# shichaoy/pop_up_slam

Hardware: AMD Instinct MI355X
Metric: graph-solve iters/sec + final chi2, 1k-pose/5k-edge plane graph (higher is better)
Workload: dtype f64; 1 GPU; C2 synthetic corridor: 1000 SE3 poses, 200 planes, 5000 plane edges, 999 odometry edges (BASELINE.json configs[1], seed 42); jacobian_mode=numeric, total_lm_solves=773

## Files before the change

### pop_up_slam_amd/csrc/pps_api.cpp

```cpp
#include "pps_graph.h"

using namespace pps;
using namespace pps_impl;

namespace pps {
Switches read_switches() {
  auto on = [](const char* k) { return getenv(k) != nullptr; };
  auto num = [](const char* k, long long dflt) { const char* e = getenv(k); return e && *e ? atoll(e) : dflt; };
  Switches s;
  s.k1_thread_form = on("PPS_K1_THREAD_FORM");
  {
    long long plain = num("PPS_PLAIN_SCHEDULE", 0);
    if (on("PPS_PLAIN_SCHEDULE") && plain <= 0) plain = 15;
    s.no_preassemble = (plain & 1) != 0; s.no_solve_flow = (plain & 2) != 0; s.no_root_fuse = (plain & 4) != 0; s.split_expand = (plain & 8) != 0;
  }
  s.no_spec_lin = on("PPS_NO_SPEC_LIN");
  s.no_dual = on("PPS_NO_DUAL");
  s.no_strip = on("PPS_NO_STRIP");
  s.no_incremental = on("PPS_NO_INCREMENTAL");
  s.no_incr_compact = on("PPS_NO_INCR_COMPACT");
  s.verify_upload = on("PPS_DEBUG_VERIFY_UPLOAD");
  s.multi_levels = on("PPS_MULTI_LEVELS");
  s.multi_thread_form = on("PPS_MULTI_THREAD_FORM");
  s.debug_drop_flag = (int)num("PPS_DEBUG_DROP_FLAG", 0);
  if (on("PPS_DEBUG_DROP_FLAG") && s.debug_drop_flag < 1) s.debug_drop_flag = 1;
  s.trace = (int)num("PPS_TRACE", 0);
  if (on("PPS_TRACE") && s.trace < 1) s.trace = 1;
  {
    long long tm = num("PPS_TIMING", 0);
    if (on("PPS_TIMING") && tm <= 0) tm = 7;
    s.analysis_timing = (tm & 1) != 0; s.upload_timing = (tm & 2) != 0; s.multi_timing = (tm & 8) ? 2 : ((tm & 4) ? 1 : 0);
  }
  s.multi_split = (int)num("PPS_MULTI_SPLIT", 0);
  s.multi_thread_factors = num("PPS_MULTI_THREAD_FACTORS", 120000);
  return s;
}
}

namespace pps_impl {
void report_front_trace(pps_graph* g) {
  const Analysis& A = g->an;
  std::vector<long long> tr((size_t)A.n_fronts * 8);
  (void)hipMemcpy(tr.data(), g->dev.trace, tr.size() * 8, hipMemcpyDeviceToHost);
  if (g->dev.trace_solve) {
    for (int l = A.n_levels - 1; l >= 0; l--) {
      double ph[5] = {0, 0, 0, 0, 0}, gap = 0; int n = 0, ng = 0;
// ... 562 lines not shown
```

### pop_up_slam_amd/csrc/pps_device.h

```cpp
#pragma once

#include <hip/hip_runtime.h>

#include <cstdint>

#include "pps_cost.h"

namespace pps {

struct DevGraph {
  int n_pose = 0, n_plane = 0, pose_ld = 0, plane_ld = 0;
  double *pose_est = nullptr, *pose_lin = nullptr;
  double *plane_est = nullptr, *plane_lin = nullptr;
  int *pose_voff = nullptr, *plane_voff = nullptr;
  int n_obs = 0, n_odo = 0, n_pp = 0, n_lp = 0;
  int obs_ld = 0, odo_ld = 0, pp_ld = 0, lp_ld = 0;
  int *obs_pose = nullptr, *obs_plane = nullptr; double *obs_meas = nullptr, *obs_w = nullptr;
  int n_obs_fixed = 0; double* obs_ray = nullptr;
  int *odo_a = nullptr, *odo_b = nullptr;         double *odo_meas = nullptr, *odo_w = nullptr;
  int *pp_pose = nullptr;                          double *pp_meas = nullptr, *pp_w = nullptr;
  int *lp_plane = nullptr;                         double *lp_meas = nullptr, *lp_w = nullptr;
  double* J = nullptr;
  int64_t joff_obs = 0, joff_odo = 0, joff_pp = 0, joff_lp = 0;
  double* P = nullptr;
// ... 37 lines not shown
  double* chi2_partials = nullptr;
  int chi2_blocks = 0;
  double* dn_partials = nullptr;
  unsigned int* ticket = nullptr;
  double* result_dev = nullptr;
  long long* trace = nullptr;
  int trace_solve = 0;
  int no_strip = 0;
  unsigned sw = 0;
  double step_ac[4] = {0, 0, 0, 0};
  double* gwork = nullptr;
  int64_t gwork_stride = 0;
};

constexpr double kStatusInternal = 64.0;
enum : unsigned { SW_K1_THREAD_FORM = 1u, SW_NO_SOLVE_FLOW = 2u, SW_NO_ROOT_FUSE = 4u, SW_DEBUG_DROP_FLAG = 8u, SW_DEBUG_DROP_XFLAG = 16u };
struct Switches {
  bool k1_thread_form = false;
  bool no_preassemble = false;
  bool no_solve_flow = false;
  bool no_root_fuse = false;
  bool split_expand = false;
  bool no_spec_lin = false;
  bool no_dual = false;
  bool no_strip = false;
  bool no_incremental = false;
  bool no_incr_compact = false;
  bool verify_upload = false;
  bool multi_levels = false, multi_thread_form = false;
  int debug_drop_flag = 0;
  int trace = 0;
  bool analysis_timing = false, upload_timing = false;
  int multi_timing = 0;
  int multi_split = 0;
  long long multi_thread_factors = 120000;
  unsigned dev_bits() const {
    return (k1_thread_form ? SW_K1_THREAD_FORM : 0u) | (no_solve_flow ? SW_NO_SOLVE_FLOW : 0u) | (no_root_fuse ? SW_NO_ROOT_FUSE : 0u) |
           (debug_drop_flag == 1 ? SW_DEBUG_DROP_FLAG : 0u) | (debug_drop_flag == 2 ? SW_DEBUG_DROP_XFLAG : 0u);
  }
};
Switches read_switches();

struct LinGuard {
  const double* chi[2];
  const double* pose[2];
  const double* plane[2];
  double error;
  int on, single;
  int want = -1;
};

struct SpecLin {
  double *J, *P, *H, *Hf;
// ... 14 lines not shown
hipError_t launch_linearize(const DevGraph& d, int mode, bool at_estimate, hipStream_t st, const LinGuard* guard = nullptr, hipEvent_t ev0 = nullptr,
                            hipEvent_t ev1 = nullptr);
hipError_t launch_hblocks(const DevGraph& d, hipStream_t st, const LinGuard* guard = nullptr, bool products = true);
bool k1_lane_form(const DevGraph& d, int mode);
bool k1_products(const DevGraph& d, int mode);
hipError_t launch_factor_level(const DevGraph& d, int level_begin, int level_count, int level_max_front, double lambda,
                               hipStream_t st);
hipError_t launch_backsolve_level(const DevGraph& d, int level_begin, int level_count, hipStream_t st);
struct DualAlt {
  double *L, *U, *delta, *result_dev, *chi2_partials, *dn_partials;
  unsigned int* ticket;
  double lambda;
};
hipError_t launch_band_all(const DevGraph& d, const DualAlt* alt, int n_groups, int nwaves_factor, int nwaves_solve, int max_front, int max_panel,
                           int max_group_fronts, double lambda, int epoch, hipStream_t st, hipEvent_t ev0 = nullptr, hipEvent_t ev1 = nullptr);
int band_all_solve_waves(int max_panel, int max_group_fronts);
hipError_t launch_band_factor(const DevGraph& d, int grp_begin, int grp_count, int nwaves, int max_front, double lambda, hipStream_t st,
                              hipEvent_t ev0 = nullptr, hipEvent_t ev1 = nullptr, bool pre = false);
hipError_t launch_band_solve(const DevGraph& d, int grp_begin, int grp_count, int nwaves, int max_panel, int max_group_fronts, hipStream_t st,
                             const DualAlt* alt = nullptr);
hipError_t launch_band_factor_dual(const DevGraph& d, const DualAlt& alt, int grp_begin, int grp_count, int nwaves, int max_front, double lambda,
                                   hipStream_t st, hipEvent_t ev0 = nullptr, hipEvent_t ev1 = nullptr, bool pre = false);
bool band_root_fusable(const DevGraph& d, int grp_count, int max_front);
hipError_t launch_band_root(const DevGraph& d, const DualAlt* alt, int grp, int nwaves_factor, int nwaves_solve, int max_front, int max_panel,
                            int max_group_fronts, double lambda, hipStream_t st, hipEvent_t ev0 = nullptr, hipEvent_t ev1 = nullptr,
                            bool pre = false);
hipError_t launch_trial_dual(const DevGraph& d, const DualAlt& alt, const double* base_pose, const double* base_plane, double* out_pose0,
                             double* out_plane0, double* out_pose1, double* out_plane1, double* host_result0, double seq0, double* host_result1,
                             double seq1, hipStream_t st, int n_trials = 2);
hipError_t launch_trial_lin(const DevGraph& d, const DualAlt& alt, const SpecLin& sl, const double* base_pose, const double* base_plane, double* out_pose0,
// ... 94 lines not shown
```

### pop_up_slam_amd/csrc/pps_k3.hip

```cpp
#include <algorithm>
#include <atomic>
#include <cstdlib>

#include <hip/hip_ext.h>

#include "pps_kcommon.h"
#include "pps_regtile.h"
#include "pps_front_reg.h"

namespace pps {


constexpr int kLdsLimitBytes = 160 * 1024 - 1024;

int lds_front_limit() {
  int fa = 1;
  while ((size_t)(fa + 1) * ((fa + 1) | 1) * 8 <= (size_t)kLdsLimitBytes) fa++;
  return fa - 1;
}

template <bool USE_LDS>
__global__ __launch_bounds__(256) void k_front_factor(DevGraph d, int level_begin, double lambda) {
  extern __shared__ double lds[];
  const int s = d.level_fronts[level_begin + blockIdx.x];
// ... 1010 lines not shown
    if ((size_t)pws * want * sizeof(double) + flow_fixed <= (size_t)kLdsLimitBytes) nw = want; else flow = false;
  }
  const size_t bf = (size_t)pwf * nw * sizeof(double);
  const size_t bs = flow ? (size_t)pws * nw * sizeof(double) + flow_fixed : ((size_t)pws * nw + (size_t)max_group_fronts * kBandMaxRows) * sizeof(double);
  const size_t bytes = bf > bs ? bf : bs;
  const DualAlt a2 = alt ? *alt : DualAlt{};
  if (pre && flow) PPS_LAUNCH_EV(ev0, ev1, (k_band_root<true, true>), dim3(1, alt ? 2 : 1), dim3(64 * nw), bytes, st, d, a2, grp, lambda, pwf, pws, max_group_fronts);
  else if (pre) PPS_LAUNCH_EV(ev0, ev1, (k_band_root<true, false>), dim3(1, alt ? 2 : 1), dim3(64 * nw), bytes, st, d, a2, grp, lambda, pwf, pws, max_group_fronts);
  else if (flow) PPS_LAUNCH_EV(ev0, ev1, (k_band_root<false, true>), dim3(1, alt ? 2 : 1), dim3(64 * nw), bytes, st, d, a2, grp, lambda, pwf, pws, max_group_fronts);
  else PPS_LAUNCH_EV(ev0, ev1, (k_band_root<false, false>), dim3(1, alt ? 2 : 1), dim3(64 * nw), bytes, st, d, a2, grp, lambda, pwf, pws, max_group_fronts);
  return hipGetLastError();
}

hipError_t launch_band_all(const DevGraph& d, const DualAlt* alt, int n_groups, int nwaves_factor, int nwaves_solve, int max_front, int max_panel,
                           int max_group_fronts, double lambda, int epoch, hipStream_t st, hipEvent_t ev0, hipEvent_t ev1) {
  { const hipError_t e = ensure_band_attrs(); if (e != hipSuccess) return e; }
  const int pwf = (int)(band_lds_bytes(max_front, true) / sizeof(double)), pws = (int)(band_solve_lds_bytes(max_panel) / sizeof(double));
  const DualAlt a2 = alt ? *alt : DualAlt{};
  PPS_LAUNCH_EV(ev0, ev1, k_band_factor_all, dim3(n_groups, alt ? 2 : 1), dim3(64 * nwaves_factor), (size_t)pwf * nwaves_factor * sizeof(double), st, d, a2, lambda, pwf, epoch);
  const size_t fixed = ((size_t)max_group_fronts * kBandMaxRows + (size_t)(max_group_fronts + 1) / 2) * sizeof(double);
  PPS_LAUNCH(k_band_solve_all, dim3(n_groups, alt ? 2 : 1), dim3(64 * nwaves_solve), (size_t)pws * nwaves_solve * sizeof(double) + fixed, st, d, a2, n_groups, pws, max_group_fronts, epoch);
  return hipGetLastError();
}
int band_all_solve_waves(int max_panel, int max_group_fronts) {
  const size_t per_wave = band_solve_lds_bytes(max_panel);
  const size_t fixed = ((size_t)max_group_fronts * kBandMaxRows + (size_t)(max_group_fronts + 1) / 2) * sizeof(double);
  const size_t room = (size_t)kLdsLimitBytes > fixed ? ((size_t)kLdsLimitBytes - fixed) / per_wave : 0;
  return (int)std::min<size_t>(std::min<size_t>(12, (size_t)max_group_fronts), room);
}

__global__ __launch_bounds__(64) void k_front_solve(DevGraph d, int level_begin) {
  __shared__ double t[256];
  const int s = d.level_fronts[level_begin + blockIdx.x];
  const int p = d.f_p[s], b = d.f_b[s], f = p + b;
  const double* __restrict__ Lp = d.L + d.f_Loff[s];
  const int* __restrict__ bi = d.bidx + d.f_bidx_off[s];
// ... 340 lines not shown
```

### pop_up_slam_amd/csrc/pps_k4.hip

```cpp
#include <algorithm>
#include <cstdlib>

#include <hip/hip_ext.h>

#include "pps_geom.h"
#include "pps_kcommon.h"
#include "pps_k1_body.h"
#include "pps_k4_body.h"

namespace pps {

template <bool TRIAL>
__device__ __forceinline__ void body_retract(const DevGraph& d, double* __restrict__ pose_lin, double* __restrict__ pose_est,
                                             double* __restrict__ plane_lin, double* __restrict__ plane_est, int bx, double* red) {
  const int i = bx * blockDim.x + threadIdx.x;
  double dn = 0.0;
  if (i < d.n_pose) {
    double p[7], o[7], dl[6];
    load_pose(pose_lin, d.pose_ld, i, p);
    const int off = d.pose_voff[i];
#pragma unroll
    for (int k = 0; k < 6; k++) { dl[k] = d.delta[off + k]; dn += dl[k] * dl[k]; }
    pose_exmap(p, dl, o);
    if (TRIAL) {
// ... 40 lines not shown
}
hipError_t launch_retract_apply(const DevGraph& d, hipStream_t st) {
  const int n = d.n_pose + d.n_plane;
  if (n == 0) return hipSuccess;
  PPS_LAUNCH(k_retract<false>, dim3(cdiv(n, 256)), dim3(256), 0, st, d);
  return hipGetLastError();
}

__global__ __launch_bounds__(kChiBlock) void k_chi2(DevGraph d, const double* __restrict__ pose,
                                                    const double* __restrict__ plane, int nb_obs, int nb_odo, int nb_pp,
                                                    int n_dn, double* __restrict__ out, double seq) {
  body_chi2(d, pose, plane, nb_obs, nb_odo, nb_pp, n_dn, out, seq, blockIdx.x, gridDim.x);
}

__device__ __forceinline__ void body_retract_to(const DevGraph& d, const double* __restrict__ base_pose, const double* __restrict__ base_plane,
                                                double* __restrict__ out_pose, double* __restrict__ out_plane, int bx, double* red) {
  const int i = bx * blockDim.x + threadIdx.x;
  double dn = 0.0;
  if (i < d.n_pose) {
    double p[7], o[7], dl[6];
    load_pose(base_pose, d.pose_ld, i, p);
    const int off = d.pose_voff[i];
#pragma unroll
    for (int k = 0; k < 6; k++) { dl[k] = d.delta[off + k]; dn += dl[k] * dl[k]; }
    pose_exmap(p, dl, o);
#pragma unroll
    for (int k = 0; k < 7; k++) out_pose[(size_t)k * d.pose_ld + i] = o[k];
  } else if (i < d.n_pose + d.n_plane) {
    const int l = i - d.n_pose;
    double p[4], o[4], dl[3];
    load_plane(base_plane, d.plane_ld, l, p);
    const int off = d.plane_voff[l];
#pragma unroll
    for (int k = 0; k < 3; k++) { dl[k] = d.delta[off + k]; dn += dl[k] * dl[k]; }
    plane_exmap(p, dl, o);
#pragma unroll
    for (int k = 0; k < 4; k++) out_plane[(size_t)k * d.plane_ld + l] = o[k];
  }
#pragma unroll
  for (int o2 = 32; o2 > 0; o2 >>= 1) dn += __shfl_down(dn, o2, 64);
  if ((threadIdx.x & 63) == 0) red[threadIdx.x >> 6] = dn;
  __syncthreads();
  if (threadIdx.x == 0) d.dn_partials[bx] = red[0] + red[1] + red[2] + red[3];
}

__global__ __launch_bounds__(kChiBlock) void k_trial_dual(DevGraph d, DualAlt alt, const double* __restrict__ base_pose, const double* __restrict__ base_plane,
                                                          double* __restrict__ out_pose, double* __restrict__ out_plane, double* __restrict__ out_pose1,
                                                          double* __restrict__ out_plane1, int nb_ret, int nb_obs, int nb_odo, int nb_pp, int nb_chi,
                                                          double* __restrict__ out, double seq, double* __restrict__ out1, double seq1) {
  if (blockIdx.y) {
    d.delta = alt.delta; d.chi2_partials = alt.chi2_partials; d.dn_partials = alt.dn_partials; d.ticket = alt.ticket; d.result_dev = alt.result_dev;
    out_pose = out_pose1; out_plane = out_plane1; out = out1; seq = seq1;
  }
  const int total = nb_ret + nb_chi;
  if ((int)blockIdx.x >= nb_ret) {
    body_chi2<true, true>(d, base_pose, base_plane, nb_obs, nb_odo, nb_pp, nb_ret, out, seq, (int)blockIdx.x - nb_ret, nb_chi, total);
    return;
  }
// ... 32 lines not shown
                                                         double* __restrict__ out, double seq, double* __restrict__ out1, double seq1, int lb_obs, int lb_odo, int lb_pp, int apply) {
  static_assert(kChiBlock == kLanesPerBlock, "one block size for the trial blocks and the lane-form sweep");
  const int total = nb_ret + nb_chi;
  const bool sweep = (int)blockIdx.x >= 2 * total;
  const int y = sweep ? sl.which : ((int)blockIdx.x >= total ? 1 : 0);
  const int bx0 = sweep ? (int)blockIdx.x - 2 * total : (int)blockIdx.x - y * total;
  if (y) {
    d.delta = alt.delta; d.chi2_partials = alt.chi2_partials; d.dn_partials = alt.dn_partials; d.ticket = alt.ticket; d.result_dev = alt.result_dev;
    out_pose = out_pose1; out_plane = out_plane1; out = out1; seq = seq1;
  }
  if (sweep) {
    d.J = sl.J; d.P = sl.P; d.H = sl.H; d.Hf = sl.Hf;
    body_linearize_lanes(d, base_pose, base_plane, lb_obs, lb_odo, lb_pp, bx0, apply != 0);
    return;
  }
  if (bx0 >= nb_ret) {
    body_chi2<true, true>(d, base_pose, base_plane, nb_obs, nb_odo, nb_pp, nb_ret, out, seq, bx0 - nb_ret, nb_chi, total);
    return;
  }
  __shared__ double red[4];
  body_retract_to(d, base_pose, base_plane, out_pose, out_plane, bx0, red);
  __shared__ bool last;
  if (threadIdx.x == 0) {
    __builtin_amdgcn_fence(__ATOMIC_RELEASE, "agent");
    asm volatile("s_waitcnt vmcnt(0)" ::: "memory");
    last = atomicAdd(d.ticket, 1u) == (unsigned int)(total - 1);
  }
  __syncthreads();
  if (!last) return;
  if (threadIdx.x == 0) __builtin_amdgcn_fence(__ATOMIC_ACQUIRE, "agent");
  __syncthreads();
  chi2_finish(d, nb_chi, nb_ret, out, seq);
  if (threadIdx.x == 0) *d.ticket = 0u;
}

int trial_lin_waves(const DevGraph& d) {
  const int nb = cdiv(d.n_obs, kChiBlock) + cdiv(d.n_odo, kChiBlock) + cdiv(d.n_pp, kChiBlock) + cdiv(d.n_lp, kChiBlock) + cdiv(d.n_pose + d.n_plane, 256);
  const int lb = cdiv(d.n_obs_fixed, kObsPerBlock) + cdiv(d.n_odo, kFactorsPerBlock) + cdiv(d.n_pp, kFactorsPerBlock) + cdiv(d.n_lp, kFactorsPerBlock);
  return (2 * nb + lb) * (kChiBlock / 64);
}
bool trial_lin_ok(const DevGraph& d, int mode) { return k1_lane_form(d, mode) && d.n_obs == d.n_obs_fixed && d.P != nullptr; }

hipError_t launch_trial_lin(const DevGraph& d, const DualAlt& alt, const SpecLin& sl, const double* base_pose, const double* base_plane, double* out_pose0,
                            double* out_plane0, double* out_pose1, double* out_plane1, double* host_result0, double seq0, double* host_result1,
                            double seq1, hipStream_t st, hipEvent_t ev0, hipEvent_t ev1) {
  const int n = d.n_pose + d.n_plane;
  const int nb_obs = cdiv(d.n_obs, kChiBlock), nb_odo = cdiv(d.n_odo, kChiBlock), nb_pp = cdiv(d.n_pp, kChiBlock), nb_lp = cdiv(d.n_lp, kChiBlock);
// ... 180 lines not shown
```

### pop_up_slam_amd/csrc/pps_k4_body.h

```cpp
#pragma once
#include "pps_cost.h"
#include "pps_geom.h"
#include "pps_kcommon.h"

namespace pps {

constexpr int kChiBlock = 256;

__device__ __forceinline__ void chi2_finish(const DevGraph& d, int nb, int n_dn, double* __restrict__ out, double seq) {
  double cs = 0.0, dn = 0.0;
  for (int i = threadIdx.x; i < nb; i += kChiBlock) cs += __hip_atomic_load(&d.chi2_partials[i], __ATOMIC_RELAXED, __HIP_MEMORY_SCOPE_AGENT);
  for (int i = threadIdx.x; i < n_dn; i += kChiBlock) dn += __hip_atomic_load(&d.dn_partials[i], __ATOMIC_RELAXED, __HIP_MEMORY_SCOPE_AGENT);
#pragma unroll
  for (int o = 32; o > 0; o >>= 1) { cs += __shfl_down(cs, o, 64); dn += __shfl_down(dn, o, 64); }
  __shared__ double red2[2][kChiBlock / 64];
  if ((threadIdx.x & 63) == 0) { red2[0][threadIdx.x >> 6] = cs; red2[1][threadIdx.x >> 6] = dn; }
  __syncthreads();
  if (threadIdx.x == 0) {
    double a = 0.0, b2 = 0.0;
    for (int k = 0; k < kChiBlock / 64; k++) { a += red2[0][k]; b2 += red2[1][k]; }
    const double npd = __hip_atomic_load(&d.result_dev[2], __ATOMIC_RELAXED, __HIP_MEMORY_SCOPE_AGENT);
    d.result_dev[0] = a; d.result_dev[1] = b2; d.result_dev[2] = 0.0;
    out[0] = a; out[1] = b2; out[2] = npd;
    __hip_atomic_store(&out[3], seq, __ATOMIC_RELEASE, __HIP_MEMORY_SCOPE_SYSTEM);
  }
}

template <bool TICKET = true, bool APPLY = false, bool ROBUST = false>
__device__ __forceinline__ void body_chi2(const DevGraph& d, const double* __restrict__ pose,
                                          const double* __restrict__ plane, int nb_obs, int nb_odo, int nb_pp,
                                          int n_dn, double* __restrict__ out, double seq, int bx, int nb, int total_blocks = 0, const CostFn& cost = CostFn{}) {
  __shared__ double red[kChiBlock / 64];
  int b = bx;
  double s = 0.0;
  if (b < nb_obs) {
    const int i = b * kChiBlock + threadIdx.x;
    if (i < d.n_obs) {
      double pz[7], pl[4], ms[4], w[6], e[3], r[3];
      fetch_pose<APPLY>(d, pose, d.obs_pose[i], pz);
      fetch_plane<APPLY>(d, plane, d.obs_plane[i], pl);
      if (i < d.n_obs_fixed) load_soa<4>(d.obs_meas, d.obs_ld, i, ms);
      else {
        double ray[6];
        load_soa<6>(d.obs_ray, d.n_obs - d.n_obs_fixed, i - d.n_obs_fixed, ray);
        repop_wall_plane(pz, ray, ms);
      }
// ... 44 lines not shown
      s = r[0] * r[0] + r[1] * r[1] + r[2] * r[2];
    }
  }
#pragma unroll
  for (int o = 32; o > 0; o >>= 1) s += __shfl_down(s, o, 64);
  if ((threadIdx.x & 63) == 0) red[threadIdx.x >> 6] = s;
  __syncthreads();
  if (!TICKET) {
    if (threadIdx.x == 0) { double t = 0.0; for (int k = 0; k < kChiBlock / 64; k++) t += red[k]; d.chi2_partials[bx] = t; }
    return;
  }
  __shared__ bool last;
  if (threadIdx.x == 0) {
    double t = 0.0;
    for (int k = 0; k < kChiBlock / 64; k++) t += red[k];
    d.chi2_partials[bx] = t;
    __builtin_amdgcn_fence(__ATOMIC_RELEASE, "agent");
    asm volatile("s_waitcnt vmcnt(0)" ::: "memory");
    last = atomicAdd(d.ticket, 1u) == (unsigned int)((total_blocks > 0 ? total_blocks : nb) - 1);
  }
  __syncthreads();
  if (!last) return;
  if (threadIdx.x == 0) __builtin_amdgcn_fence(__ATOMIC_ACQUIRE, "agent");
  __syncthreads();
  chi2_finish(d, nb, n_dn, out, seq);
  if (threadIdx.x == 0) *d.ticket = 0u;
}

}
```

### pop_up_slam_amd/csrc/pps_lm.h

```cpp
#pragma once
#include <cmath>
#include <cstdio>
#include <vector>

#include "../../include/pps.h"

namespace pps_impl {

struct LmSink {
  const pps_props* prop;
  std::vector<double>*tr_lambda, *tr_chi2;
  std::vector<int>* tr_acc;
  pps_stats* stats;
  bool verbose;
};

enum class LmVerdict { Rejected, Accepted, Converged };

constexpr const char* kLmNotPdMessage = "normal equations not positive definite at the last LM trial";

struct LmControl {
  double lambda, error = 0.0, dnorm = 0.0;
  int num_iter = 0;
  bool last_notpd = false;
  int n_notpd = 0;

  explicit LmControl(const pps_props& p) : lambda(p.lm_lambda0) {}

  bool running(const pps_props& p) const { return (p.max_iterations <= 0 || num_iter < p.max_iterations) && dnorm > p.epsilon2 && error > p.epsilon_abs; }

  void take_step(const double* rec) {
    dnorm = std::sqrt(rec[1]);
    last_notpd = rec[2] != 0.0;
    n_notpd += last_notpd ? 1 : 0;
  }

  __attribute__((always_inline)) LmVerdict judge(const LmSink& s, double error_new) {
    const pps_props& p = *s.prop;
    num_iter++;
    const double error_diff = error - error_new;
    const bool accepted = error_diff > 0.;
    s.tr_lambda->push_back(lambda); s.tr_chi2->push_back(error_new); s.tr_acc->push_back(accepted ? 1 : 0);
    if (s.verbose) fprintf(stderr, "LM Iteration %d: (lambda=%g) %s %.12g\n", num_iter, lambda, accepted ? "residual:" : "rejected", error_new);
    if (!accepted) {
      s.stats->lm_trials_rejected++;
      lambda *= p.lm_lambda_factor;
      return LmVerdict::Rejected;
    }
    s.stats->lm_trials_accepted++;
    const bool converged = error_diff < p.epsilon_rel * error;
    error = error_new;
    if (converged) return LmVerdict::Converged;
    lambda /= p.lm_lambda_factor;
    return LmVerdict::Accepted;
  }

  int finish(const LmSink& s, int* iterations) const {
    pps_stats& st = *s.stats;
    st.lm_iterations = num_iter;
    st.chi2_final = error; st.lambda_final = lambda; st.last_delta_norm = dnorm;
    st.lm_trials_notpd = n_notpd;
    if (iterations) *iterations = num_iter;
    return last_notpd ? PPS_ENOTPD : PPS_OK;
  }
};

}
```

### pop_up_slam_amd/csrc/pps_solve.cpp

```cpp
#include "pps_graph.h"

using namespace pps;
using namespace pps_impl;

namespace pps_impl {

struct PhaseTimer {
  pps_graph* g; double* acc; bool on;
  PhaseTimer(pps_graph* g_, double* a) : g(g_), acc(a), on(g_->profiling >= 2) { if (on) (void)hipEventRecord(g->ev[0], g->stream); }
  ~PhaseTimer() {
    if (!on) return;
    (void)hipEventRecord(g->ev[1], g->stream);
    (void)hipEventSynchronize(g->ev[1]);
    float ms = 0;
    (void)hipEventElapsedTime(&ms, g->ev[0], g->ev[1]);
    *acc += 1e-3 * ms;
  }
};

int do_linearize(pps_graph* g, const LinGuard* guard = nullptr) {
  if (g->profiling == 1) {
    if (g->k1_used + 2 > (int)g->k1_events.size()) {
      for (int k = 0; k < 2; k++) { hipEvent_t e; HIP_TRY(g, hipEventCreate(&e)); g->k1_events.push_back(e); }
    }
    g->k1_skip.resize(g->k1_events.size() / 2, 0);
    g->k1_skip[g->k1_used / 2] = 0;
    HIP_TRY(g, lin_launch(g, g->props.jacobian_mode, false, guard, g->k1_events[g->k1_used], g->k1_events[g->k1_used + 1]));
    g->k1_used += 2;
  } else
  { PhaseTimer t(g, &g->stats.t_linearize); HIP_TRY(g, lin_launch(g, g->props.jacobian_mode, false, guard)); }
  { PhaseTimer t(g, &g->stats.t_assemble); HIP_TRY(g, launch_hblocks(g->dev, g->stream, guard, k1_products(g->dev, g->props.jacobian_mode))); }
  if (!guard) g->stats.n_linearize++;
  return PPS_OK;
}

static int enqueue_factor_solve(pps_graph* g, const DevGraph& dv, const DualAlt* alt, double lambda, hipStream_t st_, bool events) {
  const Analysis& A = g->an;
  if (g->k3_all) {
    hipEvent_t e0 = nullptr, e1 = nullptr;
    if (events) {
      if (g->fk_used + 2 > (int)g->fk_events.size()) for (int k = 0; k < 2; k++) { hipEvent_t e; HIP_TRY(g, hipEventCreate(&e)); g->fk_events.push_back(e); }
      e0 = g->fk_events[g->fk_used]; e1 = g->fk_events[g->fk_used + 1]; g->fk_used += 2;
    }
    g->k3_epoch = g->k3_epoch >= (1 << 30) ? 1 : g->k3_epoch + 1;
    HIP_TRY(g, launch_band_all(dv, alt, A.n_groups, g->k3_nw_factor, g->k3_nw_solve, g->k3_max_front, g->k3_max_panel, g->k3_max_grp, lambda, g->k3_epoch, st_, e0, e1));
    return PPS_OK;
  }
  const int top = A.n_stages - 1;
  const bool fuse = top >= 0 && band_root_fusable(dv, A.stage_grp_off[top + 1] - A.stage_grp_off[top], A.stage_max_front[top]);
  for (int st = 0; st < A.n_stages; st++) {
    hipEvent_t e0 = nullptr, e1 = nullptr;
    if (events) {
      if (g->fk_used + 2 > (int)g->fk_events.size()) for (int k = 0; k < 2; k++) { hipEvent_t e; HIP_TRY(g, hipEventCreate(&e)); g->fk_events.push_back(e); }
      e0 = g->fk_events[g->fk_used]; e1 = g->fk_events[g->fk_used + 1]; g->fk_used += 2;
    }
    const int g0 = A.stage_grp_off[st], ng = A.stage_grp_off[st + 1] - g0;
    const bool pre = st < (int)g->stage_pre.size() && g->stage_pre[st] != 0;
    if (fuse && st == top)
      HIP_TRY(g, launch_band_root(dv, alt, g0, g->stage_nw_factor[st], g->stage_nw_solve[st], A.stage_max_front[st], g->stage_max_panel[st],
                                  g->stage_max_grp_fronts[st], lambda, st_, e0, e1, pre));
    else if (alt) HIP_TRY(g, launch_band_factor_dual(dv, *alt, g0, ng, g->stage_nw_factor[st], A.stage_max_front[st], lambda, st_, e0, e1, pre));
    else HIP_TRY(g, launch_band_factor(dv, g0, ng, g->stage_nw_factor[st], A.stage_max_front[st], lambda, st_, e0, e1, pre));
  }
  for (int st = fuse ? top - 1 : top; st >= 0; st--)
    HIP_TRY(g, launch_band_solve(dv, A.stage_grp_off[st], A.stage_grp_off[st + 1] - A.stage_grp_off[st], g->stage_nw_solve[st],
                                 g->stage_max_panel[st], g->stage_max_grp_fronts[st], st_, alt));
  return PPS_OK;
}

int do_solve_on(pps_graph* g, const DevGraph& dv, double lambda, hipStream_t st_) { return enqueue_factor_solve(g, dv, nullptr, lambda, st_, false); }
// ... 269 lines not shown
    const SpecLin sl{g->spec_J, g->spec_P, g->spec_H, g->spec_Hf, pred_launched};
    hipEvent_t e0 = nullptr, e1 = nullptr;
    fused_pair = -1;
    if (g->profiling == 1) {
      if (g->k1_used + 2 > (int)g->k1_events.size()) for (int k = 0; k < 2; k++) { hipEvent_t e; HIP_TRY(g, hipEventCreate(&e)); g->k1_events.push_back(e); }
      g->k1_skip.resize(g->k1_events.size() / 2, 0);
      fused_pair = g->k1_used / 2;
      g->k1_skip[fused_pair] = 1;
      e0 = g->k1_events[g->k1_used]; e1 = g->k1_events[g->k1_used + 1]; g->k1_used += 2;
    }
    HIP_TRY(g, launch_trial_lin(d, alt, sl, d.pose_lin, d.plane_lin, t_pose[0], t_plane[0], t_pose[1], t_plane[1], slot[0], s0, slot[1], s1, g->stream, e0, e1));
    const LinGuard gd{{d.result_dev, g->spec_result}, {nullptr, nullptr}, {nullptr, nullptr}, lm.error, error_known ? 1 : 0, use_alt ? 0 : 1, pred_launched};
    HIP_TRY(g, launch_hblocks_spec(d, sl, g->stream, &gd));
    return PPS_OK;
  };
  auto enqueue_dual = [&](double lam) -> int {
    DualAlt alt{g->spec_L, g->spec_U, g->spec_delta, g->spec_result, g->spec_chi2_partials, g->spec_dn_partials, g->spec_ticket,
                lam * prop.lm_lambda_factor};
    have_next = use_alt;
    const int n_trials = use_alt ? 2 : 1;
    { const int rc2 = enqueue_factor_solve(g, d, use_alt ? &alt : nullptr, lam, g->stream, g->profiling == 1); if (rc2 != PPS_OK) return rc2; }
    g->stats.n_factorize += n_trials;
    g->seq += 1.0; seqs[0] = g->seq;
    g->seq2 += 1.0; seqs[1] = g->seq2;
    if (fuse_lin) return enqueue_trial_lin(alt, seqs[0], seqs[1]);
    HIP_TRY(g, launch_trial_dual(d, alt, d.pose_lin, d.plane_lin, t_pose[0], t_plane[0], t_pose[1], t_plane[1], slot[0], seqs[0], slot[1], seqs[1],
                                 g->stream, n_trials));
    return PPS_OK;
  };
  rc = do_linearize(g); if (rc != PPS_OK) return rc;
  g->seq += 1.0;
  const double seq0 = g->seq;
  HIP_TRY(g, launch_chi2(d, false, slot0, seq0, g->stream));
  const bool spec_lin = !g->sw.no_spec_lin && !fuse_lin && !adaptive;
  int spec_pair = -1;
  auto enqueue_spec_lin = [&](double err) -> int {
// ... 1 lines not shown
    LinGuard gd{{d.result_dev, g->spec_result}, {t_pose[0], t_pose[1]}, {t_plane[0], t_plane[1]}, err, 1, have_next ? 0 : 1};
    spec_pair = g->profiling == 1 ? g->k1_used / 2 : -1;
    return do_linearize(g, &gd);
  };
  auto drop_spec_lin = [&]() { if (spec_pair >= 0 && (size_t)spec_pair < g->k1_skip.size()) g->k1_skip[spec_pair] = 1; spec_pair = -1; };
  rc = enqueue_dual(lm.lambda); if (rc != PPS_OK) return rc;
  rc = wait_result(g, slot0, seq0); if (rc != PPS_OK) return rc;
  lm.error = slot0[0]; error_known = true;
  g->stats.chi2_initial = lm.error;
  rc = enqueue_spec_lin(lm.error); if (rc != PPS_OK) return rc;
  rc = wait_result(g, slot[0], seqs[0]); if (rc != PPS_OK) return rc;
  int cur = 0;
  lm.take_step(slot[0]);
  bool trial_taken = false;
  while (lm.running(prop)) {
    const LmVerdict v = lm.judge(sink, slot[cur][0]);
    if (v == LmVerdict::Converged) { trial_taken = true; break; }
    if (v == LmVerdict::Accepted) {
      if (adaptive) use_alt = cur != 0;
      pred = cur;
      std::swap(d.pose_lin, t_pose[cur]); std::swap(d.plane_lin, t_plane[cur]);
      if (fuse_lin && cur == pred_launched) {
        std::swap(d.J, g->spec_J); std::swap(d.P, g->spec_P); std::swap(d.H, g->spec_H); std::swap(d.Hf, g->spec_Hf);
        g->stats.n_linearize++;
        if (fused_pair >= 0 && (size_t)fused_pair < g->k1_skip.size()) g->k1_skip[fused_pair] = 0;
      }
      else if (fuse_lin) { rc = do_linearize(g); if (rc != PPS_OK) return rc; }
      else if (spec_lin) { g->stats.n_linearize++; spec_pair = -1; }
      else { rc = do_linearize(g); if (rc != PPS_OK) return rc; }
      rc = enqueue_dual(lm.lambda); if (rc != PPS_OK) return rc;
      rc = enqueue_spec_lin(lm.error); if (rc != PPS_OK) return rc;
      cur = 0;
      rc = wait_result(g, slot[0], seqs[0]); if (rc != PPS_OK) return rc;
    } else {
      if (have_next) {
        cur = 1; have_next = false;
        rc = wait_result(g, slot[1], seqs[1]); if (rc != PPS_OK) return rc;
      } else {
        drop_spec_lin();
        if (adaptive) use_alt = true;
        rc = enqueue_dual(lm.lambda); if (rc != PPS_OK) return rc;
        rc = enqueue_spec_lin(lm.error); if (rc != PPS_OK) return rc;
        cur = 0;
        rc = wait_result(g, slot[0], seqs[0]); if (rc != PPS_OK) return rc;
      }
    }
    lm.take_step(slot[cur]);
  }
  drop_spec_lin();
  if (trial_taken) { std::swap(d.pose_lin, t_pose[cur]); std::swap(d.plane_lin, t_plane[cur]); }
  d.pose_est = d.pose_lin; d.plane_est = d.plane_lin;
  d.pose_lin = t_pose[0]; d.plane_lin = t_plane[0];
  g->spec_pose = t_pose[1]; g->spec_plane = t_plane[1];
  return end_lm_solve(g, lm, sink, iterations, t0);
}

static int lm_solve(pps_graph* g, int* iterations) {
  const double t0 = now_s();
  begin_solve(g);
  int rc = prepare_solve(g);
  if (rc != PPS_OK) return rc;
  if (g->use_band && g->profiling < 2 && !g->dev.trace && !g->sw.no_dual && !robust(g)) return lm_solve_dual(g, iterations, t0);
  const pps_props& prop = g->props;
  if (!g->status_clean) HIP_TRY(g, launch_clear_status(g->dev, g->stream));
// ... 99 lines not shown
```

Baseline: 17090 LM iters/s.

## Defer LM bookkeeping past factor launch and lighten chi2 result publishing

Splits the LM judge into a decision step and a deferred record step, so the trace and stats bookkeeping runs after the band-factor kernel is launched rather than before it. The band_all launch is split into a precomputed plan plus separate factor and solve launches, so the host starts the GPU work sooner on the critical path. On the device side, the trial and chi2 kernels publish partial sums through relaxed atomic exchanges instead of stores plus release fences, raise wave priority, and write the host-visible result with relaxed stores ordered by a waitcnt. This trades formal memory-ordering guarantees for lower fence latency. An optional timing mode reports the host gap between recording a trial and launching the factor kernel.

Result: faster. 17410 LM iters/s (median of 6 runs) (+1.9%).

```diff
diff --git a/pop_up_slam_amd/csrc/pps_api.cpp b/pop_up_slam_amd/csrc/pps_api.cpp
--- a/pop_up_slam_amd/csrc/pps_api.cpp
+++ b/pop_up_slam_amd/csrc/pps_api.cpp
@@ -16,6 +16,8 @@
   }
   s.no_spec_lin = on("PPS_NO_SPEC_LIN");
   s.no_dual = on("PPS_NO_DUAL");
+  s.lm_plain_host = on("PPS_LM_PLAIN_HOST");
+  s.no_early_record = on("PPS_NO_EARLY_RECORD");
   s.no_strip = on("PPS_NO_STRIP");
   s.no_incremental = on("PPS_NO_INCREMENTAL");
   s.no_incr_compact = on("PPS_NO_INCR_COMPACT");
@@ -30,6 +32,7 @@
     long long tm = num("PPS_TIMING", 0);
     if (on("PPS_TIMING") && tm <= 0) tm = 7;
     s.analysis_timing = (tm & 1) != 0; s.upload_timing = (tm & 2) != 0; s.multi_timing = (tm & 8) ? 2 : ((tm & 4) ? 1 : 0);
+    s.lm_timing = (tm & 16) != 0;
   }
   s.multi_split = (int)num("PPS_MULTI_SPLIT", 0);
   s.multi_thread_factors = num("PPS_MULTI_THREAD_FACTORS", 120000);
diff --git a/pop_up_slam_amd/csrc/pps_device.h b/pop_up_slam_amd/csrc/pps_device.h
--- a/pop_up_slam_amd/csrc/pps_device.h
+++ b/pop_up_slam_amd/csrc/pps_device.h
@@ -75,7 +75,7 @@
 };
 
 constexpr double kStatusInternal = 64.0;
-enum : unsigned { SW_K1_THREAD_FORM = 1u, SW_NO_SOLVE_FLOW = 2u, SW_NO_ROOT_FUSE = 4u, SW_DEBUG_DROP_FLAG = 8u, SW_DEBUG_DROP_XFLAG = 16u };
+enum : unsigned { SW_K1_THREAD_FORM = 1u, SW_NO_SOLVE_FLOW = 2u, SW_NO_ROOT_FUSE = 4u, SW_DEBUG_DROP_FLAG = 8u, SW_DEBUG_DROP_XFLAG = 16u, SW_NO_EARLY_RECORD = 32u };
 struct Switches {
   bool k1_thread_form = false;
   bool no_preassemble = false;
@@ -84,6 +84,8 @@
   bool split_expand = false;
   bool no_spec_lin = false;
   bool no_dual = false;
+  bool no_early_record = false;
+  bool lm_plain_host = false;
   bool no_strip = false;
   bool no_incremental = false;
   bool no_incr_compact = false;
@@ -91,13 +93,14 @@
   bool multi_levels = false, multi_thread_form = false;
   int debug_drop_flag = 0;
   int trace = 0;
-  bool analysis_timing = false, upload_timing = false;
+  bool analysis_timing = false, upload_timing = false, lm_timing = false;
   int multi_timing = 0;
   int multi_split = 0;
   long long multi_thread_factors = 120000;
   unsigned dev_bits() const {
     return (k1_thread_form ? SW_K1_THREAD_FORM : 0u) | (no_solve_flow ? SW_NO_SOLVE_FLOW : 0u) | (no_root_fuse ? SW_NO_ROOT_FUSE : 0u) |
-           (debug_drop_flag == 1 ? SW_DEBUG_DROP_FLAG : 0u) | (debug_drop_flag == 2 ? SW_DEBUG_DROP_XFLAG : 0u);
+           (debug_drop_flag == 1 ? SW_DEBUG_DROP_FLAG : 0u) | (debug_drop_flag == 2 ? SW_DEBUG_DROP_XFLAG : 0u) |
+           (no_early_record ? SW_NO_EARLY_RECORD : 0u);
   }
 };
 Switches read_switches();
@@ -142,6 +145,11 @@
 };
 hipError_t launch_band_all(const DevGraph& d, const DualAlt* alt, int n_groups, int nwaves_factor, int nwaves_solve, int max_front, int max_panel,
                            int max_group_fronts, double lambda, int epoch, hipStream_t st, hipEvent_t ev0 = nullptr, hipEvent_t ev1 = nullptr);
+struct BandAllPlan { int n_groups, nw_factor, nw_solve, pwf, pws, max_group_fronts; size_t lds_factor, lds_solve; };
+hipError_t band_all_plan(int n_groups, int nwaves_factor, int nwaves_solve, int max_front, int max_panel, int max_group_fronts, BandAllPlan* p);
+hipError_t launch_band_all_factor(const DevGraph& d, const DualAlt* alt, const BandAllPlan& p, double lambda, int epoch, hipStream_t st,
+                                  hipEvent_t ev0 = nullptr, hipEvent_t ev1 = nullptr);
+hipError_t launch_band_all_solve(const DevGraph& d, const DualAlt* alt, const BandAllPlan& p, int epoch, hipStream_t st);
 int band_all_solve_waves(int max_panel, int max_group_fronts);
 hipError_t launch_band_factor(const DevGraph& d, int grp_begin, int grp_count, int nwaves, int max_front, double lambda, hipStream_t st,
                               hipEvent_t ev0 = nullptr, hipEvent_t ev1 = nullptr, bool pre = false);
diff --git a/pop_up_slam_amd/csrc/pps_k3.hip b/pop_up_slam_amd/csrc/pps_k3.hip
--- a/pop_up_slam_amd/csrc/pps_k3.hip
+++ b/pop_up_slam_amd/csrc/pps_k3.hip
@@ -1048,12 +1048,29 @@
 
 hipError_t launch_band_all(const DevGraph& d, const DualAlt* alt, int n_groups, int nwaves_factor, int nwaves_solve, int max_front, int max_panel,
                            int max_group_fronts, double lambda, int epoch, hipStream_t st, hipEvent_t ev0, hipEvent_t ev1) {
+  BandAllPlan p;
+  { const hipError_t e = band_all_plan(n_groups, nwaves_factor, nwaves_solve, max_front, max_panel, max_group_fronts, &p); if (e != hipSuccess) return e; }
+  { const hipError_t e = launch_band_all_factor(d, alt, p, lambda, epoch, st, ev0, ev1); if (e != hipSuccess) return e; }
+  return launch_band_all_solve(d, alt, p, epoch, st);
+}
+hipError_t band_all_plan(int n_groups, int nwaves_factor, int nwaves_solve, int max_front, int max_panel, int max_group_fronts, BandAllPlan* p) {
   { const hipError_t e = ensure_band_attrs(); if (e != hipSuccess) return e; }
-  const int pwf = (int)(band_lds_bytes(max_front, true) / sizeof(double)), pws = (int)(band_solve_lds_bytes(max_panel) / sizeof(double));
+  p->n_groups = n_groups; p->nw_factor = nwaves_factor; p->nw_solve = nwaves_solve; p->max_group_fronts = max_group_fronts;
+  p->pwf = (int)(band_lds_bytes(max_front, true) / sizeof(double)); p->pws = (int)(band_solve_lds_bytes(max_panel) / sizeof(double));
+  p->lds_factor = (size_t)p->pwf * nwaves_factor * sizeof(double);
+  const size_t fixed = ((size_t)max_group_fronts * kBandMaxRows + (size_t)(max_group_fronts + 1) / 2) * sizeof(double);
+  p->lds_solve = (size_t)p->pws * nwaves_solve * sizeof(double) + fixed;
+  return hipSuccess;
+}
+hipError_t launch_band_all_factor(const DevGraph& d, const DualAlt* alt, const BandAllPlan& p, double lambda, int epoch, hipStream_t st, hipEvent_t ev0,
+                                  hipEvent_t ev1) {
   const DualAlt a2 = alt ? *alt : DualAlt{};
-  PPS_LAUNCH_EV(ev0, ev1, k_band_factor_all, dim3(n_groups, alt ? 2 : 1), dim3(64 * nwaves_factor), (size_t)pwf * nwaves_factor * sizeof(double), st, d, a2, lambda, pwf, epoch);
-  const size_t fixed = ((size_t)max_group_fronts * kBandMaxRows + (size_t)(max_group_fronts + 1) / 2) * sizeof(double);
-  PPS_LAUNCH(k_band_solve_all, dim3(n_groups, alt ? 2 : 1), dim3(64 * nwaves_solve), (size_t)pws * nwaves_solve * sizeof(double) + fixed, st, d, a2, n_groups, pws, max_group_fronts, epoch);
+  PPS_LAUNCH_EV(ev0, ev1, k_band_factor_all, dim3(p.n_groups, alt ? 2 : 1), dim3(64 * p.nw_factor), p.lds_factor, st, d, a2, lambda, p.pwf, epoch);
+  return hipGetLastError();
+}
+hipError_t launch_band_all_solve(const DevGraph& d, const DualAlt* alt, const BandAllPlan& p, int epoch, hipStream_t st) {
+  const DualAlt a2 = alt ? *alt : DualAlt{};
+  PPS_LAUNCH(k_band_solve_all, dim3(p.n_groups, alt ? 2 : 1), dim3(64 * p.nw_solve), p.lds_solve, st, d, a2, p.n_groups, p.pws, p.max_group_fronts, epoch);
   return hipGetLastError();
 }
 int band_all_solve_waves(int max_panel, int max_group_fronts) {
diff --git a/pop_up_slam_amd/csrc/pps_k4.hip b/pop_up_slam_amd/csrc/pps_k4.hip
--- a/pop_up_slam_amd/csrc/pps_k4.hip
+++ b/pop_up_slam_amd/csrc/pps_k4.hip
@@ -78,7 +78,7 @@
 }
 
 __device__ __forceinline__ void body_retract_to(const DevGraph& d, const double* __restrict__ base_pose, const double* __restrict__ base_plane,
-                                                double* __restrict__ out_pose, double* __restrict__ out_plane, int bx, double* red) {
+                                                double* __restrict__ out_pose, double* __restrict__ out_plane, int bx, double* red, bool light = false) {
   const int i = bx * blockDim.x + threadIdx.x;
   double dn = 0.0;
   if (i < d.n_pose) {
@@ -105,7 +105,10 @@
   for (int o2 = 32; o2 > 0; o2 >>= 1) dn += __shfl_down(dn, o2, 64);
   if ((threadIdx.x & 63) == 0) red[threadIdx.x >> 6] = dn;
   __syncthreads();
-  if (threadIdx.x == 0) d.dn_partials[bx] = red[0] + red[1] + red[2] + red[3];
+  if (threadIdx.x == 0) {
+    const double t = red[0] + red[1] + red[2] + red[3];
+    if (light) publish_partial(&d.dn_partials[bx], t); else d.dn_partials[bx] = t;
+  }
 }
 
 __global__ __launch_bounds__(kChiBlock) void k_trial_dual(DevGraph d, DualAlt alt, const double* __restrict__ base_pose, const double* __restrict__ base_plane,
@@ -168,15 +171,17 @@
     body_linearize_lanes(d, base_pose, base_plane, lb_obs, lb_odo, lb_pp, bx0, apply != 0);
     return;
   }
+  const bool light = (d.sw & SW_NO_EARLY_RECORD) == 0;
+  if (light) __builtin_amdgcn_s_setprio(3);
   if (bx0 >= nb_ret) {
-    body_chi2<true, true>(d, base_pose, base_plane, nb_obs, nb_odo, nb_pp, nb_ret, out, seq, bx0 - nb_ret, nb_chi, total);
+    body_chi2<true, true>(d, base_pose, base_plane, nb_obs, nb_odo, nb_pp, nb_ret, out, seq, bx0 - nb_ret, nb_chi, total, CostFn{}, light);
     return;
   }
   __shared__ double red[4];
-  body_retract_to(d, base_pose, base_plane, out_pose, out_plane, bx0, red);
+  body_retract_to(d, base_pose, base_plane, out_pose, out_plane, bx0, red, light);
   __shared__ bool last;
   if (threadIdx.x == 0) {
-    __builtin_amdgcn_fence(__ATOMIC_RELEASE, "agent");
+    if (!light) __builtin_amdgcn_fence(__ATOMIC_RELEASE, "agent");
     asm volatile("s_waitcnt vmcnt(0)" ::: "memory");
     last = atomicAdd(d.ticket, 1u) == (unsigned int)(total - 1);
   }
@@ -184,7 +189,7 @@
   if (!last) return;
   if (threadIdx.x == 0) __builtin_amdgcn_fence(__ATOMIC_ACQUIRE, "agent");
   __syncthreads();
-  chi2_finish(d, nb_chi, nb_ret, out, seq);
+  chi2_finish(d, nb_chi, nb_ret, out, seq, light);
   if (threadIdx.x == 0) *d.ticket = 0u;
 }
 
diff --git a/pop_up_slam_amd/csrc/pps_k4_body.h b/pop_up_slam_amd/csrc/pps_k4_body.h
--- a/pop_up_slam_amd/csrc/pps_k4_body.h
+++ b/pop_up_slam_amd/csrc/pps_k4_body.h
@@ -7,7 +7,14 @@
 
 constexpr int kChiBlock = 256;
 
-__device__ __forceinline__ void chi2_finish(const DevGraph& d, int nb, int n_dn, double* __restrict__ out, double seq) {
+__device__ __forceinline__ void publish_partial(double* p, double v) {
+  const unsigned long long old = __hip_atomic_exchange(reinterpret_cast<unsigned long long*>(p), (unsigned long long)__double_as_longlong(v),
+                                                       __ATOMIC_RELAXED, __HIP_MEMORY_SCOPE_AGENT);
+  asm volatile("" ::"v"(old));
+}
+
+__device__ __forceinline__ void chi2_finish(const DevGraph& d, int nb, int n_dn, double* __restrict__ out, double seq, bool light = false) {
+  const double npd = threadIdx.x == 0 ? __hip_atomic_load(&d.result_dev[2], __ATOMIC_RELAXED, __HIP_MEMORY_SCOPE_AGENT) : 0.0;
   double cs = 0.0, dn = 0.0;
   for (int i = threadIdx.x; i < nb; i += kChiBlock) cs += __hip_atomic_load(&d.chi2_partials[i], __ATOMIC_RELAXED, __HIP_MEMORY_SCOPE_AGENT);
   for (int i = threadIdx.x; i < n_dn; i += kChiBlock) dn += __hip_atomic_load(&d.dn_partials[i], __ATOMIC_RELAXED, __HIP_MEMORY_SCOPE_AGENT);
@@ -19,8 +26,15 @@
   if (threadIdx.x == 0) {
     double a = 0.0, b2 = 0.0;
     for (int k = 0; k < kChiBlock / 64; k++) { a += red2[0][k]; b2 += red2[1][k]; }
-    const double npd = __hip_atomic_load(&d.result_dev[2], __ATOMIC_RELAXED, __HIP_MEMORY_SCOPE_AGENT);
     d.result_dev[0] = a; d.result_dev[1] = b2; d.result_dev[2] = 0.0;
+    if (light) {
+      __hip_atomic_store(&out[0], a, __ATOMIC_RELAXED, __HIP_MEMORY_SCOPE_SYSTEM);
+      __hip_atomic_store(&out[1], b2, __ATOMIC_RELAXED, __HIP_MEMORY_SCOPE_SYSTEM);
+      __hip_atomic_store(&out[2], npd, __ATOMIC_RELAXED, __HIP_MEMORY_SCOPE_SYSTEM);
+      asm volatile("s_waitcnt vmcnt(0)" ::: "memory");
+      __hip_atomic_store(&out[3], seq, __ATOMIC_RELAXED, __HIP_MEMORY_SCOPE_SYSTEM);
+      return;
+    }
     out[0] = a; out[1] = b2; out[2] = npd;
     __hip_atomic_store(&out[3], seq, __ATOMIC_RELEASE, __HIP_MEMORY_SCOPE_SYSTEM);
   }
@@ -29,7 +43,7 @@
 template <bool TICKET = true, bool APPLY = false, bool ROBUST = false>
 __device__ __forceinline__ void body_chi2(const DevGraph& d, const double* __restrict__ pose,
                                           const double* __restrict__ plane, int nb_obs, int nb_odo, int nb_pp,
-                                          int n_dn, double* __restrict__ out, double seq, int bx, int nb, int total_blocks = 0, const CostFn& cost = CostFn{}) {
+                                          int n_dn, double* __restrict__ out, double seq, int bx, int nb, int total_blocks = 0, const CostFn& cost = CostFn{}, bool light = false) {
   __shared__ double red[kChiBlock / 64];
   int b = bx;
   double s = 0.0;
@@ -104,8 +118,8 @@
   if (threadIdx.x == 0) {
     double t = 0.0;
     for (int k = 0; k < kChiBlock / 64; k++) t += red[k];
-    d.chi2_partials[bx] = t;
-    __builtin_amdgcn_fence(__ATOMIC_RELEASE, "agent");
+    if (light) publish_partial(&d.chi2_partials[bx], t);
+    else { d.chi2_partials[bx] = t; __builtin_amdgcn_fence(__ATOMIC_RELEASE, "agent"); }
     asm volatile("s_waitcnt vmcnt(0)" ::: "memory");
     last = atomicAdd(d.ticket, 1u) == (unsigned int)((total_blocks > 0 ? total_blocks : nb) - 1);
   }
@@ -113,7 +127,7 @@
   if (!last) return;
   if (threadIdx.x == 0) __builtin_amdgcn_fence(__ATOMIC_ACQUIRE, "agent");
   __syncthreads();
-  chi2_finish(d, nb, n_dn, out, seq);
+  chi2_finish(d, nb, n_dn, out, seq, light);
   if (threadIdx.x == 0) *d.ticket = 0u;
 }
 
diff --git a/pop_up_slam_amd/csrc/pps_lm.h b/pop_up_slam_amd/csrc/pps_lm.h
--- a/pop_up_slam_amd/csrc/pps_lm.h
+++ b/pop_up_slam_amd/csrc/pps_lm.h
@@ -35,24 +35,32 @@
     n_notpd += last_notpd ? 1 : 0;
   }
 
-  __attribute__((always_inline)) LmVerdict judge(const LmSink& s, double error_new) {
-    const pps_props& p = *s.prop;
+  struct Trial { double lambda, chi2; int iter; bool accepted; };
+  __attribute__((always_inline)) LmVerdict decide(const pps_props& p, double error_new, Trial* t) {
     num_iter++;
     const double error_diff = error - error_new;
     const bool accepted = error_diff > 0.;
-    s.tr_lambda->push_back(lambda); s.tr_chi2->push_back(error_new); s.tr_acc->push_back(accepted ? 1 : 0);
-    if (s.verbose) fprintf(stderr, "LM Iteration %d: (lambda=%g) %s %.12g\n", num_iter, lambda, accepted ? "residual:" : "rejected", error_new);
+    *t = Trial{lambda, error_new, num_iter, accepted};
     if (!accepted) {
-      s.stats->lm_trials_rejected++;
       lambda *= p.lm_lambda_factor;
       return LmVerdict::Rejected;
     }
-    s.stats->lm_trials_accepted++;
     const bool converged = error_diff < p.epsilon_rel * error;
     error = error_new;
     if (converged) return LmVerdict::Converged;
     lambda /= p.lm_lambda_factor;
     return LmVerdict::Accepted;
+  }
+  static void note(const LmSink& s, const Trial& t) {
+    s.tr_lambda->push_back(t.lambda); s.tr_chi2->push_back(t.chi2); s.tr_acc->push_back(t.accepted ? 1 : 0);
+    if (s.verbose) fprintf(stderr, "LM Iteration %d: (lambda=%g) %s %.12g\n", t.iter, t.lambda, t.accepted ? "residual:" : "rejected", t.chi2);
+    if (t.accepted) s.stats->lm_trials_accepted++; else s.stats->lm_trials_rejected++;
+  }
+  __attribute__((always_inline)) LmVerdict judge(const LmSink& s, double error_new) {
+    Trial t;
+    const LmVerdict v = decide(*s.prop, error_new, &t);
+    note(s, t);
+    return v;
   }
 
   int finish(const LmSink& s, int* iterations) const {
diff --git a/pop_up_slam_amd/csrc/pps_solve.cpp b/pop_up_slam_amd/csrc/pps_solve.cpp
--- a/pop_up_slam_amd/csrc/pps_solve.cpp
+++ b/pop_up_slam_amd/csrc/pps_solve.cpp
@@ -34,14 +34,19 @@
   return PPS_OK;
 }
 
+static int take_factor_events(pps_graph* g, bool events, hipEvent_t* e0, hipEvent_t* e1) {
+  *e0 = *e1 = nullptr;
+  if (!events) return PPS_OK;
+  if (g->fk_used + 2 > (int)g->fk_events.size()) for (int k = 0; k < 2; k++) { hipEvent_t e; HIP_TRY(g, hipEventCreate(&e)); g->fk_events.push_back(e); }
+  *e0 = g->fk_events[g->fk_used]; *e1 = g->fk_events[g->fk_used + 1]; g->fk_used += 2;
+  return PPS_OK;
+}
+
 static int enqueue_factor_solve(pps_graph* g, const DevGraph& dv, const DualAlt* alt, double lambda, hipStream_t st_, bool events) {
   const Analysis& A = g->an;
   if (g->k3_all) {
-    hipEvent_t e0 = nullptr, e1 = nullptr;
-    if (events) {
-      if (g->fk_used + 2 > (int)g->fk_events.size()) for (int k = 0; k < 2; k++) { hipEvent_t e; HIP_TRY(g, hipEventCreate(&e)); g->fk_events.push_back(e); }
-      e0 = g->fk_events[g->fk_used]; e1 = g->fk_events[g->fk_used + 1]; g->fk_used += 2;
-    }
+    hipEvent_t e0, e1;
+    { const int rc = take_factor_events(g, events, &e0, &e1); if (rc != PPS_OK) return rc; }
     g->k3_epoch = g->k3_epoch >= (1 << 30) ? 1 : g->k3_epoch + 1;
     HIP_TRY(g, launch_band_all(dv, alt, A.n_groups, g->k3_nw_factor, g->k3_nw_solve, g->k3_max_front, g->k3_max_panel, g->k3_max_grp, lambda, g->k3_epoch, st_, e0, e1));
     return PPS_OK;
@@ -49,11 +54,8 @@
   const int top = A.n_stages - 1;
   const bool fuse = top >= 0 && band_root_fusable(dv, A.stage_grp_off[top + 1] - A.stage_grp_off[top], A.stage_max_front[top]);
   for (int st = 0; st < A.n_stages; st++) {
-    hipEvent_t e0 = nullptr, e1 = nullptr;
-    if (events) {
-      if (g->fk_used + 2 > (int)g->fk_events.size()) for (int k = 0; k < 2; k++) { hipEvent_t e; HIP_TRY(g, hipEventCreate(&e)); g->fk_events.push_back(e); }
-      e0 = g->fk_events[g->fk_used]; e1 = g->fk_events[g->fk_used + 1]; g->fk_used += 2;
-    }
+    hipEvent_t e0, e1;
+    { const int rc = take_factor_events(g, events, &e0, &e1); if (rc != PPS_OK) return rc; }
     const int g0 = A.stage_grp_off[st], ng = A.stage_grp_off[st + 1] - g0;
     const bool pre = st < (int)g->stage_pre.size() && g->stage_pre[st] != 0;
     if (fuse && st == top)
@@ -353,12 +355,42 @@
     HIP_TRY(g, launch_hblocks_spec(d, sl, g->stream, &gd));
     return PPS_OK;
   };
+  const bool plain_host = g->sw.lm_plain_host;
+  BandAllPlan plan{};
+  const bool planned = !plain_host && g->k3_all;
+  if (planned) HIP_TRY(g, band_all_plan(A.n_groups, g->k3_nw_factor, g->k3_nw_solve, g->k3_max_front, g->k3_max_panel, g->k3_max_grp, &plan));
+  struct PendingNote {
+    const LmSink& s; LmControl::Trial t{}; bool owed = false;
+    void flush() { if (owed) { LmControl::note(s, t); owed = false; } }
+    ~PendingNote() { flush(); }
+  } pending{sink};
+  const bool lm_timing = g->sw.lm_timing;
+  double t_rec = 0.0, rt_pre = 0.0, rt_call = 0.0, rt_relin = 0.0; int rt_n = 0, rt_n_relin = 0; bool relin = false;
+  auto rt_note = [&](double t_pre) {
+    if (!lm_timing || t_rec <= 0.0) return;
+    const double t = now_s();
+    if (relin) { rt_relin += t - t_rec; rt_n_relin++; } else { rt_pre += t_pre - t_rec; rt_call += t - t_pre; rt_n++; }
+    t_rec = 0.0; relin = false;
+  };
   auto enqueue_dual = [&](double lam) -> int {
     DualAlt alt{g->spec_L, g->spec_U, g->spec_delta, g->spec_result, g->spec_chi2_partials, g->spec_dn_partials, g->spec_ticket,
                 lam * prop.lm_lambda_factor};
     have_next = use_alt;
     const int n_trials = use_alt ? 2 : 1;
-    { const int rc2 = enqueue_factor_solve(g, d, use_alt ? &alt : nullptr, lam, g->stream, g->profiling == 1); if (rc2 != PPS_OK) return rc2; }
+    const double t_pre = lm_timing ? now_s() : 0.0;
+    if (planned) {
+      hipEvent_t e0, e1;
+      { const int rc2 = take_factor_events(g, g->profiling == 1, &e0, &e1); if (rc2 != PPS_OK) return rc2; }
+      g->k3_epoch = g->k3_epoch >= (1 << 30) ? 1 : g->k3_epoch + 1;
+      HIP_TRY(g, launch_band_all_factor(d, use_alt ? &alt : nullptr, plan, lam, g->k3_epoch, g->stream, e0, e1));
+      rt_note(t_pre);
+      pending.flush();
+      HIP_TRY(g, launch_band_all_solve(d, use_alt ? &alt : nullptr, plan, g->k3_epoch, g->stream));
+    } else {
+      const int rc2 = enqueue_factor_solve(g, d, use_alt ? &alt : nullptr, lam, g->stream, g->profiling == 1); if (rc2 != PPS_OK) return rc2;
+      rt_note(t_pre);
+      pending.flush();
+    }
     g->stats.n_factorize += n_trials;
     g->seq += 1.0; seqs[0] = g->seq;
     g->seq2 += 1.0; seqs[1] = g->seq2;
@@ -390,7 +422,10 @@
   lm.take_step(slot[0]);
   bool trial_taken = false;
   while (lm.running(prop)) {
-    const LmVerdict v = lm.judge(sink, slot[cur][0]);
+    if (lm_timing) t_rec = now_s();
+    LmVerdict v;
+    if (plain_host) v = lm.judge(sink, slot[cur][0]);
+    else { v = lm.decide(prop, slot[cur][0], &pending.t); pending.owed = true; }
     if (v == LmVerdict::Converged) { trial_taken = true; break; }
     if (v == LmVerdict::Accepted) {
       if (adaptive) use_alt = cur != 0;
@@ -401,7 +436,7 @@
         g->stats.n_linearize++;
         if (fused_pair >= 0 && (size_t)fused_pair < g->k1_skip.size()) g->k1_skip[fused_pair] = 0;
       }
-      else if (fuse_lin) { rc = do_linearize(g); if (rc != PPS_OK) return rc; }
+      else if (fuse_lin) { relin = true; rc = do_linearize(g); if (rc != PPS_OK) return rc; }
       else if (spec_lin) { g->stats.n_linearize++; spec_pair = -1; }
       else { rc = do_linearize(g); if (rc != PPS_OK) return rc; }
       rc = enqueue_dual(lm.lambda); if (rc != PPS_OK) return rc;
@@ -410,7 +445,8 @@
       rc = wait_result(g, slot[0], seqs[0]); if (rc != PPS_OK) return rc;
     } else {
       if (have_next) {
-        cur = 1; have_next = false;
+        cur = 1; have_next = false; t_rec = 0.0;
+        pending.flush();
         rc = wait_result(g, slot[1], seqs[1]); if (rc != PPS_OK) return rc;
       } else {
         drop_spec_lin();
@@ -424,6 +460,10 @@
     lm.take_step(slot[cur]);
   }
   drop_spec_lin();
+  pending.flush();
+  if (lm_timing && rt_n > 0)
+    fprintf(stderr, "[lm] record -> factor launch: %d launch sets, mean %.2f us before the launch call + %.2f us inside it; %d sets that relinearised first, mean %.2f us\n",
+            rt_n, 1e6 * rt_pre / rt_n, 1e6 * rt_call / rt_n, rt_n_relin, rt_n_relin ? 1e6 * rt_relin / rt_n_relin : 0.0);
   if (trial_taken) { std::swap(d.pose_lin, t_pose[cur]); std::swap(d.plane_lin, t_plane[cur]); }
   d.pose_est = d.pose_lin; d.plane_est = d.plane_lin;
   d.pose_lin = t_pose[0]; d.plane_lin = t_plane[0];
```
